# facebookresearch/actionmesh

Measured on NVIDIA H100. Metric: denoiser_steps_per_sec, higher is better.
Workload: dtype bf16

## Files before the change

actionmesh_b200/csrc/attention.cu:

```cuda
#include "common.cuh"
#include "ptx.cuh"
#include "attention.cuh"

namespace amb {

constexpr int ATT_BQ = 128;
constexpr int ATT_BK = 128;
constexpr int ATT_THREADS = 384;
constexpr int ATT_STAGES = 2;

template <int D>
struct AttnSmem {
  static constexpr int BOX_BYTES = 128 * 128;
  static constexpr int Q_BYTES = (D / 64) * BOX_BYTES;
  static constexpr int KV_BYTES = (D / 64) * BOX_BYTES;
  static constexpr int Q_OFF = 0;
  static constexpr int K_OFF = Q_BYTES;
  static constexpr int V_OFF = K_OFF + ATT_STAGES * KV_BYTES;
  static constexpr int BAR_OFF = V_OFF + ATT_STAGES * KV_BYTES;
  static constexpr int NUM_BARS = 1 + 3 * ATT_STAGES;
  static constexpr int TOTAL = BAR_OFF + NUM_BARS * 8 + 1024;
};

template <int D>
__device__ __forceinline__ void pv_k16(float* o, const uint32_t* a, uint64_t vdesc) {
  if constexpr (D == 128) wgmma_rs_n128_tb(o, a, vdesc, 1u);
  else wgmma_rs_n64_tb(o, a, vdesc, 1u);
}

template <int D>
__global__ void __launch_bounds__(ATT_THREADS, 1)
flash_attn_fwd_kernel(const __grid_constant__ CUtensorMap tmQ, const __grid_constant__ CUtensorMap tmK,
                      const __grid_constant__ CUtensorMap tmV, const AttnParams p) {
  using L = AttnSmem<D>;
  constexpr int DH = D / 64;
  extern __shared__ uint8_t smem_raw[];
  uint8_t* smem = reinterpret_cast<uint8_t*>((reinterpret_cast<uintptr_t>(smem_raw) + 1023) & ~uintptr_t(1023));
  uint64_t* q_full = reinterpret_cast<uint64_t*>(smem + L::BAR_OFF);
  uint64_t* k_full = q_full + 1;
  uint64_t* v_full = k_full + ATT_STAGES;
  uint64_t* kv_empty = v_full + ATT_STAGES;

  const int wg = __shfl_sync(0xffffffffu, threadIdx.x >> 7, 0);
  const int warp = threadIdx.x >> 5;
  const int lane = threadIdx.x & 31;
  const int q0 = blockIdx.x * ATT_BQ;
  const int head = blockIdx.y;
  const int batch = blockIdx.z;
  const int tiles_per_chunk = (p.sk_chunk + ATT_BK - 1) / ATT_BK;
  const int n_kv = p.kv_chunks * tiles_per_chunk;

  if (threadIdx.x == 0) {
    tma_prefetch_desc(&tmQ);
    tma_prefetch_desc(&tmK);
    tma_prefetch_desc(&tmV);
    mbar_init(q_full, 1);
    for (int s = 0; s < ATT_STAGES; ++s) {
      mbar_init(&k_full[s], 1);
      mbar_init(&v_full[s], 1);
      mbar_init(&kv_empty[s], 8);
    }
    fence_mbar_init();
  }
  __syncthreads();

  if (wg == 0) {
    reg_dealloc<24>();
    if (warp == 0) {
      if (elect_one()) {
        mbar_expect_tx(q_full, L::Q_BYTES);
        for (int c = 0; c < DH; ++c)
          tma_load_4d(smem + L::Q_OFF + c * L::BOX_BYTES, &tmQ, q_full, c * 64, q0, head, batch, kEvictFirst);
      }
      __syncwarp();
      int s = 0;
      uint32_t phase = 0;
      for (int j = 0; j < n_kv; ++j) {
        const int chunk = j / tiles_per_chunk;
        const int key0 = (j - chunk * tiles_per_chunk) * ATT_BK;
        mbar_wait(&kv_empty[s], phase ^ 1);
        if (elect_one()) {
          uint8_t* sk = smem + L::K_OFF + s * L::KV_BYTES;
          uint8_t* sv = smem + L::V_OFF + s * L::KV_BYTES;
          mbar_expect_tx(&k_full[s], L::KV_BYTES);
          for (int c = 0; c < DH; ++c)
            tma_load_5d(sk + c * L::BOX_BYTES, &tmK, &k_full[s], c * 64, key0, head, batch, chunk, kEvictLast);
          mbar_expect_tx(&v_full[s], L::KV_BYTES);
          for (int c = 0; c < DH; ++c)
            tma_load_5d(sv + c * L::BOX_BYTES, &tmV, &v_full[s], c * 64, key0, head, batch, chunk, kEvictLast);
        }
        __syncwarp();
        if (++s == ATT_STAGES) { s = 0; phase ^= 1; }
      }
    }
  } else {
    reg_alloc<240>();
    const int q = lane & 3;
    const int r_local = (wg - 1) * 64 + (warp & 3) * 16 + (lane >> 2);
    const uint32_t sq_addr = smem_u32(smem + L::Q_OFF) + (wg - 1) * 64 * 128;
    const uint32_t sk_addr = smem_u32(smem + L::K_OFF);
    const uint32_t sv_addr = smem_u32(smem + L::V_OFF);
    const float c = p.scale_log2;
    const int last_valid = p.sk_chunk - (tiles_per_chunk - 1) * ATT_BK;

    float o[D / 2];
#pragma unroll
    for (int i = 0; i < D / 2; ++i) o[i] = 0.f;
    float m_a = -INFINITY, m_b = -INFINITY;
    float l_a = 0.f, l_b = 0.f;

    mbar_wait(q_full, 0);
    int s = 0, jj = 0;
    uint32_t phase = 0;
    for (int j = 0; j < n_kv; ++j) {
      float sc[64];
#pragma unroll
      for (int i = 0; i < 64; ++i) sc[i] = 0.f;
      mbar_wait(&k_full[s], phase);
      wgmma_fence();
#pragma unroll
      for (int k = 0; k < D / 16; ++k) {
        const uint32_t off = (k >> 2) * L::BOX_BYTES + (k & 3) * 32;
        wgmma_ss_n128(sc, make_desc_kmajor_sw128(sq_addr + off), make_desc_kmajor_sw128(sk_addr + s * L::KV_BYTES + off), 1u);
      }
      wgmma_commit();
      wgmma_wait<0>();
#pragma unroll
      for (int i = 0; i < 64; ++i) reg_fence(sc[i]);

      if (jj == tiles_per_chunk - 1 && last_valid < ATT_BK) {
#pragma unroll
        for (int i = 0; i < 16; ++i) {
          const int key = 8 * i + 2 * q;
          if (key >= last_valid) sc[4 * i] = sc[4 * i + 2] = -INFINITY;
          if (key + 1 >= last_valid) sc[4 * i + 1] = sc[4 * i + 3] = -INFINITY;
        }
      }
      if (++jj == tiles_per_chunk) jj = 0;
      float mx_a = m_a, mx_b = m_b;
#pragma unroll
      for (int i = 0; i < 16; ++i) {
        mx_a = fmaxf(mx_a, fmaxf(sc[4 * i], sc[4 * i + 1]));
        mx_b = fmaxf(mx_b, fmaxf(sc[4 * i + 2], sc[4 * i + 3]));
      }
      mx_a = fmaxf(mx_a, __shfl_xor_sync(0xffffffffu, mx_a, 1));
      mx_b = fmaxf(mx_b, __shfl_xor_sync(0xffffffffu, mx_b, 1));
      mx_a = fmaxf(mx_a, __shfl_xor_sync(0xffffffffu, mx_a, 2));
      mx_b = fmaxf(mx_b, __shfl_xor_sync(0xffffffffu, mx_b, 2));
      const float al_a = ex2_approx((m_a - mx_a) * c), al_b = ex2_approx((m_b - mx_b) * c);
      m_a = mx_a;
      m_b = mx_b;
      const float mb_a = m_a * c, mb_b = m_b * c;
      uint32_t pk[32];
      float ts_a = 0.f, ts_b = 0.f;
#pragma unroll
      for (int i = 0; i < 16; ++i) {
        const float ea0 = ex2_approx(fmaf(sc[4 * i], c, -mb_a)), ea1 = ex2_approx(fmaf(sc[4 * i + 1], c, -mb_a));
        const float eb0 = ex2_approx(fmaf(sc[4 * i + 2], c, -mb_b)), eb1 = ex2_approx(fmaf(sc[4 * i + 3], c, -mb_b));
        ts_a += ea0 + ea1;
        ts_b += eb0 + eb1;
        pk[2 * i] = pack_bf16(ea0, ea1);
        pk[2 * i + 1] = pack_bf16(eb0, eb1);
      }
      l_a = l_a * al_a + ts_a;
      l_b = l_b * al_b + ts_b;
#pragma unroll
      for (int i = 0; i < D / 8; ++i) {
        o[4 * i] *= al_a;
        o[4 * i + 1] *= al_a;
        o[4 * i + 2] *= al_b;
        o[4 * i + 3] *= al_b;
      }

      mbar_wait(&v_full[s], phase);
      wgmma_fence();
      const uint32_t vbase = sv_addr + s * L::KV_BYTES;
#pragma unroll
      for (int kk = 0; kk < ATT_BK / 16; ++kk)
        pv_k16<D>(o, pk + 4 * kk, make_desc_mnmajor_sw128(vbase + kk * 2048, L::BOX_BYTES));
      wgmma_commit();
      wgmma_wait<0>();
#pragma unroll
      for (int i = 0; i < D / 2; ++i) reg_fence(o[i]);
      __syncwarp();
      if (lane == 0) mbar_arrive(&kv_empty[s]);
      if (++s == ATT_STAGES) { s = 0; phase ^= 1; }
    }

    l_a += __shfl_xor_sync(0xffffffffu, l_a, 1);
    l_b += __shfl_xor_sync(0xffffffffu, l_b, 1);
    l_a += __shfl_xor_sync(0xffffffffu, l_a, 2);
    l_b += __shfl_xor_sync(0xffffffffu, l_b, 2);
    const float inv_a = 1.0f / l_a, inv_b = 1.0f / l_b;
    const int qr_a = q0 + r_local, qr_b = qr_a + 8;
    __nv_bfloat16* obase = p.o + (long long)batch * p.o_stride_b + (long long)head * p.o_stride_h + 2 * q;
#pragma unroll
    for (int i = 0; i < D / 8; ++i) {
      if (qr_a < p.sq)
        *reinterpret_cast<uint32_t*>(obase + (long long)qr_a * p.o_stride_s + 8 * i) = pack_bf16(o[4 * i] * inv_a, o[4 * i + 1] * inv_a);
      if (qr_b < p.sq)
        *reinterpret_cast<uint32_t*>(obase + (long long)qr_b * p.o_stride_s + 8 * i) = pack_bf16(o[4 * i + 2] * inv_b, o[4 * i + 3] * inv_b);
    }
  }
}

template <int D>
static int launch_attn(const amb_attn_args* a, cudaStream_t stream) {
  using L = AttnSmem<D>;
  CUtensorMap tmQ, tmK, tmV;
  int r = encode_attn_maps(a, D, ATT_BQ, ATT_BK, ATT_BK, &tmQ, &tmK, &tmV);
  if (r) return r;
  const AttnParams p = make_attn_params(a);
  dim3 grid((a->sq + ATT_BQ - 1) / ATT_BQ, a->heads, a->batch);
  auto kern = flash_attn_fwd_kernel<D>;
  r = ensure_smem_optin(kern, L::TOTAL);
  if (r) return r;
  kern<<<grid, ATT_THREADS, L::TOTAL, stream>>>(tmQ, tmK, tmV, p);
  AMB_CHECK_CUDA(cudaGetLastError());
  return AMB_OK;
}

}

using namespace amb;

extern "C" int amb_flash_attn_fwd(const amb_attn_args* a, amb_stream_t stream) {
  AMB_CHECK_ARG(a && a->q && a->k && a->v && a->o, "flash_attn: null pointer");
  AMB_CHECK_ARG(a->batch > 0 && a->heads > 0 && a->sq > 0 && a->sk > 0, "flash_attn: bad shape b=%d h=%d sq=%d sk=%d",
                a->batch, a->heads, a->sq, a->sk);
  AMB_CHECK_ARG(a->head_dim == 128 || a->head_dim == 64, "flash_attn: head_dim %d unsupported (64 or 128)", a->head_dim);
  AMB_CHECK_ARG(a->q_stride_s % 8 == 0 && a->k_stride_s % 8 == 0 && a->v_stride_s % 8 == 0 && a->o_stride_s % 8 == 0 &&
                    a->q_stride_h % 8 == 0 && a->k_stride_h % 8 == 0 && a->v_stride_h % 8 == 0 && a->o_stride_h % 8 == 0 &&
                    a->q_stride_b % 8 == 0 && a->k_stride_b % 8 == 0 && a->v_stride_b % 8 == 0 && a->o_stride_b % 8 == 0,
                "flash_attn: strides must be multiples of 8 elements (16 bytes)");
  AMB_CHECK_ARG(a->kv_chunks <= 1 || (a->sk_chunk > 0 && (int64_t)a->sk_chunk * a->kv_chunks == a->sk),
                "flash_attn: kv_chunks * sk_chunk must equal sk");
  AMB_CHECK_ARG(a->batch <= 65535 && a->heads <= 65535, "flash_attn: grid limits");
  cudaStream_t s = (cudaStream_t)stream;
  if (a->head_dim == 64) return launch_attn<64>(a, s);
  return launch_attn<128>(a, s);
}
```

actionmesh_b200/csrc/ptx.cuh:

```cuda
#pragma once
#include <cstdint>
#include <cuda_runtime.h>
#include <cuda_bf16.h>

namespace amb {

__device__ __forceinline__ uint32_t smem_u32(const void* p) {
  return static_cast<uint32_t>(__cvta_generic_to_shared(p));
}
__device__ __forceinline__ uint32_t lane_id() { return threadIdx.x & 31; }

__device__ __forceinline__ bool elect_one() {
  uint32_t pred = 0;
  asm volatile(
      "{\n\t.reg .pred P;\n\t"
      "elect.sync _|P, 0xffffffff;\n\t"
      "selp.u32 %0, 1, 0, P;\n\t}\n"
      : "=r"(pred));
  return pred != 0;
}

__device__ __forceinline__ void mbar_init(uint64_t* bar, uint32_t count) {
  asm volatile("mbarrier.init.shared::cta.b64 [%0], %1;" ::"r"(smem_u32(bar)), "r"(count) : "memory");
}
__device__ __forceinline__ void fence_mbar_init() {
  asm volatile("fence.mbarrier_init.release.cluster;" ::: "memory");
}
__device__ __forceinline__ void fence_proxy_async_smem() {
  asm volatile("fence.proxy.async.shared::cta;" ::: "memory");
}
__device__ __forceinline__ void mbar_expect_tx(uint64_t* bar, uint32_t bytes) {
  asm volatile("mbarrier.arrive.expect_tx.shared::cta.b64 _, [%0], %1;" ::"r"(smem_u32(bar)), "r"(bytes)
               : "memory");
}
__device__ __forceinline__ void mbar_arrive(uint64_t* bar) {
  asm volatile("mbarrier.arrive.shared::cta.b64 _, [%0];" ::"r"(smem_u32(bar)) : "memory");
}
__device__ __forceinline__ uint32_t mbar_try_wait(uint64_t* bar, uint32_t parity) {
  uint32_t ok;
  asm volatile(
      "{\n\t.reg .pred P;\n\t"
      "mbarrier.try_wait.parity.shared::cta.b64 P, [%1], %2;\n\t"
      "selp.u32 %0, 1, 0, P;\n\t}\n"
      : "=r"(ok)
      : "r"(smem_u32(bar)), "r"(parity)
      : "memory");
  return ok;
}
__device__ __forceinline__ uint64_t globaltimer_ns() {
  uint64_t t;
  asm volatile("mov.u64 %0, %%globaltimer;" : "=l"(t));
  return t;
}
#ifndef AMB_WAIT_TIMEOUT_NS
#define AMB_WAIT_TIMEOUT_NS 4000000000ull
#endif
__device__ __forceinline__ void mbar_wait(uint64_t* bar, uint32_t parity) {
  if (mbar_try_wait(bar, parity)) return;
  uint64_t t0 = globaltimer_ns();
  uint32_t spins = 0;
  while (!mbar_try_wait(bar, parity)) {
    if ((++spins & 0xfff) == 0 && globaltimer_ns() - t0 > AMB_WAIT_TIMEOUT_NS) {
      printf("amb: mbarrier wait timeout block=(%d,%d,%d) thread=%d bar=%u parity=%u\n", blockIdx.x, blockIdx.y,
             blockIdx.z, threadIdx.x, smem_u32(bar), parity);
      __trap();
    }
  }
}

__device__ __forceinline__ void tma_prefetch_desc(const void* tmap) {
  asm volatile("prefetch.tensormap [%0];" ::"l"(reinterpret_cast<uint64_t>(tmap)) : "memory");
}
constexpr uint64_t kEvictNormal = 0x1000000000000000ull;
constexpr uint64_t kEvictFirst = 0x12F0000000000000ull;
constexpr uint64_t kEvictLast = 0x14F0000000000000ull;

__device__ __forceinline__ void tma_load_2d(void* dst, const void* tmap, uint64_t* bar, int c0, int c1,
                                            uint64_t hint) {
  asm volatile(
      "cp.async.bulk.tensor.2d.shared::cluster.global.mbarrier::complete_tx::bytes.L2::cache_hint"
      " [%0], [%1, {%3, %4}], [%2], %5;"
      :
      : "r"(smem_u32(dst)), "l"(reinterpret_cast<uint64_t>(tmap)), "r"(smem_u32(bar)), "r"(c0), "r"(c1), "l"(hint)
      : "memory");
}
__device__ __forceinline__ void tma_load_4d(void* dst, const void* tmap, uint64_t* bar, int c0, int c1, int c2,
                                            int c3, uint64_t hint) {
  asm volatile(
      "cp.async.bulk.tensor.4d.shared::cluster.global.mbarrier::complete_tx::bytes.L2::cache_hint"
      " [%0], [%1, {%3, %4, %5, %6}], [%2], %7;"
      :
      : "r"(smem_u32(dst)), "l"(reinterpret_cast<uint64_t>(tmap)), "r"(smem_u32(bar)), "r"(c0), "r"(c1), "r"(c2),
        "r"(c3), "l"(hint)
      : "memory");
}

__device__ __forceinline__ void tma_load_5d(void* dst, const void* tmap, uint64_t* bar, int c0, int c1, int c2,
                                            int c3, int c4, uint64_t hint) {
  asm volatile(
      "cp.async.bulk.tensor.5d.shared::cluster.global.mbarrier::complete_tx::bytes.L2::cache_hint"
      " [%0], [%1, {%3, %4, %5, %6, %7}], [%2], %8;"
      :
      : "r"(smem_u32(dst)), "l"(reinterpret_cast<uint64_t>(tmap)), "r"(smem_u32(bar)), "r"(c0), "r"(c1), "r"(c2),
        "r"(c3), "r"(c4), "l"(hint)
      : "memory");
}

__device__ __forceinline__ void wgmma_fence() { asm volatile("wgmma.fence.sync.aligned;" ::: "memory"); }
__device__ __forceinline__ void wgmma_commit() { asm volatile("wgmma.commit_group.sync.aligned;" ::: "memory"); }
template <int N>
__device__ __forceinline__ void wgmma_wait() {
  asm volatile("wgmma.wait_group.sync.aligned %0;" ::"n"(N) : "memory");
}
__device__ __forceinline__ void reg_fence(float& r) { asm volatile("" : "+f"(r)::"memory"); }

__device__ __forceinline__ uint64_t make_smem_desc(uint32_t saddr, uint32_t lbo_bytes, uint32_t sbo_bytes) {
  uint64_t d = 0;
  d |= static_cast<uint64_t>((saddr & 0x3FFFF) >> 4);
  d |= static_cast<uint64_t>((lbo_bytes >> 4) & 0x3FFF) << 16;
  d |= static_cast<uint64_t>((sbo_bytes >> 4) & 0x3FFF) << 32;
  d |= 1ull << 62;
  return d;
}
__device__ __forceinline__ uint64_t make_desc_kmajor_sw128(uint32_t saddr) { return make_smem_desc(saddr, 16, 1024); }
__device__ __forceinline__ uint64_t make_desc_mnmajor_sw128(uint32_t saddr, uint32_t lbo_bytes) {
  return make_smem_desc(saddr, lbo_bytes, 1024);
}

__device__ __forceinline__ void wgmma_ss_n64(float* d, uint64_t desc_a, uint64_t desc_b, uint32_t scale_d) {
  asm volatile(
      "{\n\t.reg .pred p;\n\tsetp.ne.b32 p, %34, 0;\n\t"
      "wgmma.mma_async.sync.aligned.m64n64k16.f32.bf16.bf16 {%0, %1, %2, %3, %4, %5, %6, %7, %8, %9, %10, %11, %12, %13, %14, %15, %16, %17, %18, %19, %20, %21, %22, %23, %24, %25, %26, %27, %28, %29, %30, %31}, %32, %33, p, 1, 1, 0, 0;\n\t}\n"
      : "+f"(d[0]), "+f"(d[1]), "+f"(d[2]), "+f"(d[3]), "+f"(d[4]), "+f"(d[5]), "+f"(d[6]), "+f"(d[7]), "+f"(d[8]), "+f"(d[9]), "+f"(d[10]), "+f"(d[11]), "+f"(d[12]), "+f"(d[13]), "+f"(d[14]), "+f"(d[15]), "+f"(d[16]), "+f"(d[17]), "+f"(d[18]), "+f"(d[19]), "+f"(d[20]), "+f"(d[21]), "+f"(d[22]), "+f"(d[23]), "+f"(d[24]), "+f"(d[25]), "+f"(d[26]), "+f"(d[27]), "+f"(d[28]), "+f"(d[29]), "+f"(d[30]), "+f"(d[31])
      : "l"(desc_a), "l"(desc_b), "r"(scale_d));
}
__device__ __forceinline__ void wgmma_ss_n128(float* d, uint64_t desc_a, uint64_t desc_b, uint32_t scale_d) {
  asm volatile(
      "{\n\t.reg .pred p;\n\tsetp.ne.b32 p, %66, 0;\n\t"
      "wgmma.mma_async.sync.aligned.m64n128k16.f32.bf16.bf16 {%0, %1, %2, %3, %4, %5, %6, %7, %8, %9, %10, %11, %12, %13, %14, %15, %16, %17, %18, %19, %20, %21, %22, %23, %24, %25, %26, %27, %28, %29, %30, %31, %32, %33, %34, %35, %36, %37, %38, %39, %40, %41, %42, %43, %44, %45, %46, %47, %48, %49, %50, %51, %52, %53, %54, %55, %56, %57, %58, %59, %60, %61, %62, %63}, %64, %65, p, 1, 1, 0, 0;\n\t}\n"
      : "+f"(d[0]), "+f"(d[1]), "+f"(d[2]), "+f"(d[3]), "+f"(d[4]), "+f"(d[5]), "+f"(d[6]), "+f"(d[7]), "+f"(d[8]), "+f"(d[9]), "+f"(d[10]), "+f"(d[11]), "+f"(d[12]), "+f"(d[13]), "+f"(d[14]), "+f"(d[15]), "+f"(d[16]), "+f"(d[17]), "+f"(d[18]), "+f"(d[19]), "+f"(d[20]), "+f"(d[21]), "+f"(d[22]), "+f"(d[23]), "+f"(d[24]), "+f"(d[25]), "+f"(d[26]), "+f"(d[27]), "+f"(d[28]), "+f"(d[29]), "+f"(d[30]), "+f"(d[31]), "+f"(d[32]), "+f"(d[33]), "+f"(d[34]), "+f"(d[35]), "+f"(d[36]), "+f"(d[37]), "+f"(d[38]), "+f"(d[39]), "+f"(d[40]), "+f"(d[41]), "+f"(d[42]), "+f"(d[43]), "+f"(d[44]), "+f"(d[45]), "+f"(d[46]), "+f"(d[47]), "+f"(d[48]), "+f"(d[49]), "+f"(d[50]), "+f"(d[51]), "+f"(d[52]), "+f"(d[53]), "+f"(d[54]), "+f"(d[55]), "+f"(d[56]), "+f"(d[57]), "+f"(d[58]), "+f"(d[59]), "+f"(d[60]), "+f"(d[61]), "+f"(d[62]), "+f"(d[63])
      : "l"(desc_a), "l"(desc_b), "r"(scale_d));
}
__device__ __forceinline__ void wgmma_ss_n256(float* d, uint64_t desc_a, uint64_t desc_b, uint32_t scale_d) {
  asm volatile(
      "{\n\t.reg .pred p;\n\tsetp.ne.b32 p, %130, 0;\n\t"
      "wgmma.mma_async.sync.aligned.m64n256k16.f32.bf16.bf16 {%0, %1, %2, %3, %4, %5, %6, %7, %8, %9, %10, %11, %12, %13, %14, %15, %16, %17, %18, %19, %20, %21, %22, %23, %24, %25, %26, %27, %28, %29, %30, %31, %32, %33, %34, %35, %36, %37, %38, %39, %40, %41, %42, %43, %44, %45, %46, %47, %48, %49, %50, %51, %52, %53, %54, %55, %56, %57, %58, %59, %60, %61, %62, %63, %64, %65, %66, %67, %68, %69, %70, %71, %72, %73, %74, %75, %76, %77, %78, %79, %80, %81, %82, %83, %84, %85, %86, %87, %88, %89, %90, %91, %92, %93, %94, %95, %96, %97, %98, %99, %100, %101, %102, %103, %104, %105, %106, %107, %108, %109, %110, %111, %112, %113, %114, %115, %116, %117, %118, %119, %120, %121, %122, %123, %124, %125, %126, %127}, %128, %129, p, 1, 1, 0, 0;\n\t}\n"
      : "+f"(d[0]), "+f"(d[1]), "+f"(d[2]), "+f"(d[3]), "+f"(d[4]), "+f"(d[5]), "+f"(d[6]), "+f"(d[7]), "+f"(d[8]), "+f"(d[9]), "+f"(d[10]), "+f"(d[11]), "+f"(d[12]), "+f"(d[13]), "+f"(d[14]), "+f"(d[15]), "+f"(d[16]), "+f"(d[17]), "+f"(d[18]), "+f"(d[19]), "+f"(d[20]), "+f"(d[21]), "+f"(d[22]), "+f"(d[23]), "+f"(d[24]), "+f"(d[25]), "+f"(d[26]), "+f"(d[27]), "+f"(d[28]), "+f"(d[29]), "+f"(d[30]), "+f"(d[31]), "+f"(d[32]), "+f"(d[33]), "+f"(d[34]), "+f"(d[35]), "+f"(d[36]), "+f"(d[37]), "+f"(d[38]), "+f"(d[39]), "+f"(d[40]), "+f"(d[41]), "+f"(d[42]), "+f"(d[43]), "+f"(d[44]), "+f"(d[45]), "+f"(d[46]), "+f"(d[47]), "+f"(d[48]), "+f"(d[49]), "+f"(d[50]), "+f"(d[51]), "+f"(d[52]), "+f"(d[53]), "+f"(d[54]), "+f"(d[55]), "+f"(d[56]), "+f"(d[57]), "+f"(d[58]), "+f"(d[59]), "+f"(d[60]), "+f"(d[61]), "+f"(d[62]), "+f"(d[63]), "+f"(d[64]), "+f"(d[65]), "+f"(d[66]), "+f"(d[67]), "+f"(d[68]), "+f"(d[69]), "+f"(d[70]), "+f"(d[71]), "+f"(d[72]), "+f"(d[73]), "+f"(d[74]), "+f"(d[75]), "+f"(d[76]), "+f"(d[77]), "+f"(d[78]), "+f"(d[79]), "+f"(d[80]), "+f"(d[81]), "+f"(d[82]), "+f"(d[83]), "+f"(d[84]), "+f"(d[85]), "+f"(d[86]), "+f"(d[87]), "+f"(d[88]), "+f"(d[89]), "+f"(d[90]), "+f"(d[91]), "+f"(d[92]), "+f"(d[93]), "+f"(d[94]), "+f"(d[95]), "+f"(d[96]), "+f"(d[97]), "+f"(d[98]), "+f"(d[99]), "+f"(d[100]), "+f"(d[101]), "+f"(d[102]), "+f"(d[103]), "+f"(d[104]), "+f"(d[105]), "+f"(d[106]), "+f"(d[107]), "+f"(d[108]), "+f"(d[109]), "+f"(d[110]), "+f"(d[111]), "+f"(d[112]), "+f"(d[113]), "+f"(d[114]), "+f"(d[115]), "+f"(d[116]), "+f"(d[117]), "+f"(d[118]), "+f"(d[119]), "+f"(d[120]), "+f"(d[121]), "+f"(d[122]), "+f"(d[123]), "+f"(d[124]), "+f"(d[125]), "+f"(d[126]), "+f"(d[127])
      : "l"(desc_a), "l"(desc_b), "r"(scale_d));
}
__device__ __forceinline__ void wgmma_rs_n64_tb(float* d, const uint32_t* a, uint64_t desc_b, uint32_t scale_d) {
  asm volatile(
      "{\n\t.reg .pred p;\n\tsetp.ne.b32 p, %37, 0;\n\t"
      "wgmma.mma_async.sync.aligned.m64n64k16.f32.bf16.bf16 {%0, %1, %2, %3, %4, %5, %6, %7, %8, %9, %10, %11, %12, %13, %14, %15, %16, %17, %18, %19, %20, %21, %22, %23, %24, %25, %26, %27, %28, %29, %30, %31}, {%32, %33, %34, %35}, %36, p, 1, 1, 1;\n\t}\n"
      : "+f"(d[0]), "+f"(d[1]), "+f"(d[2]), "+f"(d[3]), "+f"(d[4]), "+f"(d[5]), "+f"(d[6]), "+f"(d[7]), "+f"(d[8]), "+f"(d[9]), "+f"(d[10]), "+f"(d[11]), "+f"(d[12]), "+f"(d[13]), "+f"(d[14]), "+f"(d[15]), "+f"(d[16]), "+f"(d[17]), "+f"(d[18]), "+f"(d[19]), "+f"(d[20]), "+f"(d[21]), "+f"(d[22]), "+f"(d[23]), "+f"(d[24]), "+f"(d[25]), "+f"(d[26]), "+f"(d[27]), "+f"(d[28]), "+f"(d[29]), "+f"(d[30]), "+f"(d[31])
      : "r"(a[0]), "r"(a[1]), "r"(a[2]), "r"(a[3]), "l"(desc_b), "r"(scale_d));
}
__device__ __forceinline__ void wgmma_rs_n128_tb(float* d, const uint32_t* a, uint64_t desc_b, uint32_t scale_d) {
  asm volatile(
      "{\n\t.reg .pred p;\n\tsetp.ne.b32 p, %69, 0;\n\t"
      "wgmma.mma_async.sync.aligned.m64n128k16.f32.bf16.bf16 {%0, %1, %2, %3, %4, %5, %6, %7, %8, %9, %10, %11, %12, %13, %14, %15, %16, %17, %18, %19, %20, %21, %22, %23, %24, %25, %26, %27, %28, %29, %30, %31, %32, %33, %34, %35, %36, %37, %38, %39, %40, %41, %42, %43, %44, %45, %46, %47, %48, %49, %50, %51, %52, %53, %54, %55, %56, %57, %58, %59, %60, %61, %62, %63}, {%64, %65, %66, %67}, %68, p, 1, 1, 1;\n\t}\n"
      : "+f"(d[0]), "+f"(d[1]), "+f"(d[2]), "+f"(d[3]), "+f"(d[4]), "+f"(d[5]), "+f"(d[6]), "+f"(d[7]), "+f"(d[8]), "+f"(d[9]), "+f"(d[10]), "+f"(d[11]), "+f"(d[12]), "+f"(d[13]), "+f"(d[14]), "+f"(d[15]), "+f"(d[16]), "+f"(d[17]), "+f"(d[18]), "+f"(d[19]), "+f"(d[20]), "+f"(d[21]), "+f"(d[22]), "+f"(d[23]), "+f"(d[24]), "+f"(d[25]), "+f"(d[26]), "+f"(d[27]), "+f"(d[28]), "+f"(d[29]), "+f"(d[30]), "+f"(d[31]), "+f"(d[32]), "+f"(d[33]), "+f"(d[34]), "+f"(d[35]), "+f"(d[36]), "+f"(d[37]), "+f"(d[38]), "+f"(d[39]), "+f"(d[40]), "+f"(d[41]), "+f"(d[42]), "+f"(d[43]), "+f"(d[44]), "+f"(d[45]), "+f"(d[46]), "+f"(d[47]), "+f"(d[48]), "+f"(d[49]), "+f"(d[50]), "+f"(d[51]), "+f"(d[52]), "+f"(d[53]), "+f"(d[54]), "+f"(d[55]), "+f"(d[56]), "+f"(d[57]), "+f"(d[58]), "+f"(d[59]), "+f"(d[60]), "+f"(d[61]), "+f"(d[62]), "+f"(d[63])
      : "r"(a[0]), "r"(a[1]), "r"(a[2]), "r"(a[3]), "l"(desc_b), "r"(scale_d));
}

__device__ __forceinline__ void named_bar_sync(uint32_t id, uint32_t nthreads) {
  asm volatile("bar.sync %0, %1;" ::"r"(id), "r"(nthreads) : "memory");
}

template <int N>
__device__ __forceinline__ void reg_alloc() {
  asm volatile("setmaxnreg.inc.sync.aligned.u32 %0;" ::"n"(N));
}
template <int N>
__device__ __forceinline__ void reg_dealloc() {
  asm volatile("setmaxnreg.dec.sync.aligned.u32 %0;" ::"n"(N));
}
__device__ __forceinline__ float ex2_approx(float x) {
  float y;
  asm("ex2.approx.ftz.f32 %0, %1;" : "=f"(y) : "f"(x));
  return y;
}
__device__ __forceinline__ uint32_t pack_bf16(float lo, float hi) {
  __nv_bfloat162 v = __floats2bfloat162_rn(lo, hi);
  return *reinterpret_cast<uint32_t*>(&v);
}
__device__ __forceinline__ float2 unpack_bf16(uint32_t u) {
  __nv_bfloat162 v = *reinterpret_cast<__nv_bfloat162*>(&u);
  return __bfloat1622float2(v);
}

}
```

Measured before the change: 0.6745.

## Pipeline QK and PV wgmma across iterations with ping-pong warpgroup scheduling

```diff
diff --git a/actionmesh_b200/csrc/attention.cu b/actionmesh_b200/csrc/attention.cu
--- a/actionmesh_b200/csrc/attention.cu
+++ b/actionmesh_b200/csrc/attention.cu
@@ -18,14 +18,76 @@
   static constexpr int K_OFF = Q_BYTES;
   static constexpr int V_OFF = K_OFF + ATT_STAGES * KV_BYTES;
   static constexpr int BAR_OFF = V_OFF + ATT_STAGES * KV_BYTES;
-  static constexpr int NUM_BARS = 1 + 3 * ATT_STAGES;
+  static constexpr int NUM_BARS = 1 + 4 * ATT_STAGES;
   static constexpr int TOTAL = BAR_OFF + NUM_BARS * 8 + 1024;
 };
 
 template <int D>
-__device__ __forceinline__ void pv_k16(float* o, const uint32_t* a, uint64_t vdesc) {
-  if constexpr (D == 128) wgmma_rs_n128_tb(o, a, vdesc, 1u);
-  else wgmma_rs_n64_tb(o, a, vdesc, 1u);
+__device__ __forceinline__ void qk_issue(float* sc, uint32_t sq_addr, uint32_t sk_addr) {
+#pragma unroll
+  for (int k = 0; k < D / 16; ++k) {
+    const uint32_t off = (k >> 2) * AttnSmem<D>::BOX_BYTES + (k & 3) * 32;
+    wgmma_ss_n128(sc, make_desc_kmajor_sw128(sq_addr + off), make_desc_kmajor_sw128(sk_addr + off), k > 0 ? 1u : 0u);
+  }
+  wgmma_commit();
+}
+
+template <int D>
+__device__ __forceinline__ void pv_issue(float* o, const uint32_t* pk, uint32_t sv_addr) {
+#pragma unroll
+  for (int kk = 0; kk < ATT_BK / 16; ++kk) {
+    const uint64_t vdesc = make_desc_mnmajor_sw128(sv_addr + kk * 2048, AttnSmem<D>::BOX_BYTES);
+    if constexpr (D == 128) wgmma_rs_n128_tb(o, pk + 4 * kk, vdesc, 1u);
+    else wgmma_rs_n64_tb(o, pk + 4 * kk, vdesc, 1u);
+  }
+  wgmma_commit();
+}
+
+__device__ __forceinline__ void softmax_tile(float* sc, int valid, int q, float c, float& m_a, float& m_b, float& l_a,
+                                             float& l_b, float& al_a, float& al_b) {
+  if (valid < ATT_BK) {
+#pragma unroll
+    for (int i = 0; i < 16; ++i) {
+      const int key = 8 * i + 2 * q;
+      if (key >= valid) sc[4 * i] = sc[4 * i + 2] = -INFINITY;
+      if (key + 1 >= valid) sc[4 * i + 1] = sc[4 * i + 3] = -INFINITY;
+    }
+  }
+  float mx_a = m_a, mx_b = m_b;
+#pragma unroll
+  for (int i = 0; i < 16; ++i) {
+    mx_a = fmaxf(mx_a, fmaxf(sc[4 * i], sc[4 * i + 1]));
+    mx_b = fmaxf(mx_b, fmaxf(sc[4 * i + 2], sc[4 * i + 3]));
+  }
+  mx_a = fmaxf(mx_a, __shfl_xor_sync(0xffffffffu, mx_a, 1));
+  mx_b = fmaxf(mx_b, __shfl_xor_sync(0xffffffffu, mx_b, 1));
+  mx_a = fmaxf(mx_a, __shfl_xor_sync(0xffffffffu, mx_a, 2));
+  mx_b = fmaxf(mx_b, __shfl_xor_sync(0xffffffffu, mx_b, 2));
+  al_a = ex2_approx((m_a - mx_a) * c);
+  al_b = ex2_approx((m_b - mx_b) * c);
+  m_a = mx_a;
+  m_b = mx_b;
+  const float mb_a = m_a * c, mb_b = m_b * c;
+  float ts_a = 0.f, ts_b = 0.f;
+#pragma unroll
+  for (int i = 0; i < 16; ++i) {
+    sc[4 * i] = ex2_approx(fmaf(sc[4 * i], c, -mb_a));
+    sc[4 * i + 1] = ex2_approx(fmaf(sc[4 * i + 1], c, -mb_a));
+    sc[4 * i + 2] = ex2_approx(fmaf(sc[4 * i + 2], c, -mb_b));
+    sc[4 * i + 3] = ex2_approx(fmaf(sc[4 * i + 3], c, -mb_b));
+    ts_a += sc[4 * i] + sc[4 * i + 1];
+    ts_b += sc[4 * i + 2] + sc[4 * i + 3];
+  }
+  l_a = l_a * al_a + ts_a;
+  l_b = l_b * al_b + ts_b;
+}
+
+__device__ __forceinline__ void pack_p(uint32_t* pk, const float* sc) {
+#pragma unroll
+  for (int i = 0; i < 16; ++i) {
+    pk[2 * i] = pack_bf16(sc[4 * i], sc[4 * i + 1]);
+    pk[2 * i + 1] = pack_bf16(sc[4 * i + 2], sc[4 * i + 3]);
+  }
 }
 
 template <int D>
@@ -39,7 +101,8 @@
   uint64_t* q_full = reinterpret_cast<uint64_t*>(smem + L::BAR_OFF);
   uint64_t* k_full = q_full + 1;
   uint64_t* v_full = k_full + ATT_STAGES;
-  uint64_t* kv_empty = v_full + ATT_STAGES;
+  uint64_t* k_empty = v_full + ATT_STAGES;
+  uint64_t* v_empty = k_empty + ATT_STAGES;
 
   const int wg = __shfl_sync(0xffffffffu, threadIdx.x >> 7, 0);
   const int warp = threadIdx.x >> 5;
@@ -58,7 +121,8 @@
     for (int s = 0; s < ATT_STAGES; ++s) {
       mbar_init(&k_full[s], 1);
       mbar_init(&v_full[s], 1);
-      mbar_init(&kv_empty[s], 8);
+      mbar_init(&k_empty[s], 8);
+      mbar_init(&v_empty[s], 8);
     }
     fence_mbar_init();
   }
@@ -78,18 +142,27 @@
       for (int j = 0; j < n_kv; ++j) {
         const int chunk = j / tiles_per_chunk;
         const int key0 = (j - chunk * tiles_per_chunk) * ATT_BK;
-        mbar_wait(&kv_empty[s], phase ^ 1);
+        mbar_wait(&k_empty[s], phase ^ 1);
         if (elect_one()) {
           uint8_t* sk = smem + L::K_OFF + s * L::KV_BYTES;
-          uint8_t* sv = smem + L::V_OFF + s * L::KV_BYTES;
           mbar_expect_tx(&k_full[s], L::KV_BYTES);
           for (int c = 0; c < DH; ++c)
             tma_load_5d(sk + c * L::BOX_BYTES, &tmK, &k_full[s], c * 64, key0, head, batch, chunk, kEvictLast);
+        }
+        __syncwarp();
+        mbar_wait(&v_empty[s], phase ^ 1);
+        if (elect_one()) {
+          uint8_t* sv = smem + L::V_OFF + s * L::KV_BYTES;
           mbar_expect_tx(&v_full[s], L::KV_BYTES);
           for (int c = 0; c < DH; ++c)
             tma_load_5d(sv + c * L::BOX_BYTES, &tmV, &v_full[s], c * 64, key0, head, batch, chunk, kEvictLast);
         }
         __syncwarp();
+        if (++s == ATT_STAGES) { s = 0; phase ^= 1; }
+      }
+      for (int j = 0; j < ATT_STAGES; ++j) {
+        mbar_wait(&k_empty[s], phase ^ 1);
+        mbar_wait(&v_empty[s], phase ^ 1);
         if (++s == ATT_STAGES) { s = 0; phase ^= 1; }
       }
     }
@@ -102,68 +175,57 @@
     const uint32_t sv_addr = smem_u32(smem + L::V_OFF);
     const float c = p.scale_log2;
     const int last_valid = p.sk_chunk - (tiles_per_chunk - 1) * ATT_BK;
+    const uint32_t my_turn = wg, other_turn = 3 - wg;
 
     float o[D / 2];
 #pragma unroll
     for (int i = 0; i < D / 2; ++i) o[i] = 0.f;
     float m_a = -INFINITY, m_b = -INFINITY;
     float l_a = 0.f, l_b = 0.f;
-
-    mbar_wait(q_full, 0);
-    int s = 0, jj = 0;
+    float al_a, al_b;
+    float sc[64];
+    uint32_t pk[32];
+
+    mbar_wait_watched(q_full, 0);
+    mbar_wait_watched(&k_full[0], 0);
+    if (wg == 2) named_bar_sync(my_turn, 256);
+    wgmma_fence();
+    qk_issue<D>(sc, sq_addr, sk_addr);
+    named_bar_arrive(other_turn, 256);
+    wgmma_wait<0>();
+#pragma unroll
+    for (int i = 0; i < 64; ++i) reg_fence(sc[i]);
+    __syncwarp();
+    if (lane == 0) mbar_arrive(&k_empty[0]);
+    int jn = tiles_per_chunk == 1 ? 0 : 1;
+    softmax_tile(sc, tiles_per_chunk == 1 ? last_valid : ATT_BK, q, c, m_a, m_b, l_a, l_b, al_a, al_b);
+    pack_p(pk, sc);
+
+    int s = 0;
     uint32_t phase = 0;
-    for (int j = 0; j < n_kv; ++j) {
-      float sc[64];
-#pragma unroll
-      for (int i = 0; i < 64; ++i) sc[i] = 0.f;
-      mbar_wait(&k_full[s], phase);
+    for (int j = 0; j + 1 < n_kv; ++j) {
+      int sn = s + 1;
+      uint32_t phn = phase;
+      if (sn == ATT_STAGES) { sn = 0; phn ^= 1; }
+      mbar_wait_watched(&k_full[sn], phn);
+      mbar_wait_watched(&v_full[s], phase);
+      named_bar_sync(my_turn, 256);
       wgmma_fence();
-#pragma unroll
-      for (int k = 0; k < D / 16; ++k) {
-        const uint32_t off = (k >> 2) * L::BOX_BYTES + (k & 3) * 32;
-        wgmma_ss_n128(sc, make_desc_kmajor_sw128(sq_addr + off), make_desc_kmajor_sw128(sk_addr + s * L::KV_BYTES + off), 1u);
-      }
-      wgmma_commit();
+      qk_issue<D>(sc, sq_addr, sk_addr + sn * L::KV_BYTES);
+      pv_issue<D>(o, pk, sv_addr + s * L::KV_BYTES);
+      named_bar_arrive(other_turn, 256);
+      wgmma_wait<1>();
+#pragma unroll
+      for (int i = 0; i < 64; ++i) reg_fence(sc[i]);
+      __syncwarp();
+      if (lane == 0) mbar_arrive(&k_empty[sn]);
+      softmax_tile(sc, jn == tiles_per_chunk - 1 ? last_valid : ATT_BK, q, c, m_a, m_b, l_a, l_b, al_a, al_b);
+      if (++jn == tiles_per_chunk) jn = 0;
       wgmma_wait<0>();
 #pragma unroll
-      for (int i = 0; i < 64; ++i) reg_fence(sc[i]);
-
-      if (jj == tiles_per_chunk - 1 && last_valid < ATT_BK) {
-#pragma unroll
-        for (int i = 0; i < 16; ++i) {
-          const int key = 8 * i + 2 * q;
-          if (key >= last_valid) sc[4 * i] = sc[4 * i + 2] = -INFINITY;
-          if (key + 1 >= last_valid) sc[4 * i + 1] = sc[4 * i + 3] = -INFINITY;
-        }
-      }
-      if (++jj == tiles_per_chunk) jj = 0;
-      float mx_a = m_a, mx_b = m_b;
-#pragma unroll
-      for (int i = 0; i < 16; ++i) {
-        mx_a = fmaxf(mx_a, fmaxf(sc[4 * i], sc[4 * i + 1]));
-        mx_b = fmaxf(mx_b, fmaxf(sc[4 * i + 2], sc[4 * i + 3]));
-      }
-      mx_a = fmaxf(mx_a, __shfl_xor_sync(0xffffffffu, mx_a, 1));
-      mx_b = fmaxf(mx_b, __shfl_xor_sync(0xffffffffu, mx_b, 1));
-      mx_a = fmaxf(mx_a, __shfl_xor_sync(0xffffffffu, mx_a, 2));
-      mx_b = fmaxf(mx_b, __shfl_xor_sync(0xffffffffu, mx_b, 2));
-      const float al_a = ex2_approx((m_a - mx_a) * c), al_b = ex2_approx((m_b - mx_b) * c);
-      m_a = mx_a;
-      m_b = mx_b;
-      const float mb_a = m_a * c, mb_b = m_b * c;
-      uint32_t pk[32];
-      float ts_a = 0.f, ts_b = 0.f;
-#pragma unroll
-      for (int i = 0; i < 16; ++i) {
-        const float ea0 = ex2_approx(fmaf(sc[4 * i], c, -mb_a)), ea1 = ex2_approx(fmaf(sc[4 * i + 1], c, -mb_a));
-        const float eb0 = ex2_approx(fmaf(sc[4 * i + 2], c, -mb_b)), eb1 = ex2_approx(fmaf(sc[4 * i + 3], c, -mb_b));
-        ts_a += ea0 + ea1;
-        ts_b += eb0 + eb1;
-        pk[2 * i] = pack_bf16(ea0, ea1);
-        pk[2 * i + 1] = pack_bf16(eb0, eb1);
-      }
-      l_a = l_a * al_a + ts_a;
-      l_b = l_b * al_b + ts_b;
+      for (int i = 0; i < D / 2; ++i) reg_fence(o[i]);
+      __syncwarp();
+      if (lane == 0) mbar_arrive(&v_empty[s]);
 #pragma unroll
       for (int i = 0; i < D / 8; ++i) {
         o[4 * i] *= al_a;
@@ -171,21 +233,21 @@
         o[4 * i + 2] *= al_b;
         o[4 * i + 3] *= al_b;
       }
-
-      mbar_wait(&v_full[s], phase);
-      wgmma_fence();
-      const uint32_t vbase = sv_addr + s * L::KV_BYTES;
-#pragma unroll
-      for (int kk = 0; kk < ATT_BK / 16; ++kk)
-        pv_k16<D>(o, pk + 4 * kk, make_desc_mnmajor_sw128(vbase + kk * 2048, L::BOX_BYTES));
-      wgmma_commit();
-      wgmma_wait<0>();
-#pragma unroll
-      for (int i = 0; i < D / 2; ++i) reg_fence(o[i]);
-      __syncwarp();
-      if (lane == 0) mbar_arrive(&kv_empty[s]);
-      if (++s == ATT_STAGES) { s = 0; phase ^= 1; }
-    }
+      pack_p(pk, sc);
+      s = sn;
+      phase = phn;
+    }
+
+    mbar_wait_watched(&v_full[s], phase);
+    named_bar_sync(my_turn, 256);
+    wgmma_fence();
+    pv_issue<D>(o, pk, sv_addr + s * L::KV_BYTES);
+    if (wg == 1) named_bar_arrive(other_turn, 256);
+    wgmma_wait<0>();
+#pragma unroll
+    for (int i = 0; i < D / 2; ++i) reg_fence(o[i]);
+    __syncwarp();
+    if (lane == 0) mbar_arrive(&v_empty[s]);
 
     l_a += __shfl_xor_sync(0xffffffffu, l_a, 1);
     l_b += __shfl_xor_sync(0xffffffffu, l_b, 1);
diff --git a/actionmesh_b200/csrc/ptx.cuh b/actionmesh_b200/csrc/ptx.cuh
--- a/actionmesh_b200/csrc/ptx.cuh
+++ b/actionmesh_b200/csrc/ptx.cuh
@@ -54,6 +54,9 @@
 }
 #ifndef AMB_WAIT_TIMEOUT_NS
 #define AMB_WAIT_TIMEOUT_NS 4000000000ull
+#endif
+#ifndef AMB_WAIT_TIMEOUT_PRINT
+#define AMB_WAIT_TIMEOUT_PRINT 0
 #endif
 __device__ __forceinline__ void mbar_wait(uint64_t* bar, uint32_t parity) {
   if (mbar_try_wait(bar, parity)) return;
@@ -61,10 +64,16 @@
   uint32_t spins = 0;
   while (!mbar_try_wait(bar, parity)) {
     if ((++spins & 0xfff) == 0 && globaltimer_ns() - t0 > AMB_WAIT_TIMEOUT_NS) {
+#if AMB_WAIT_TIMEOUT_PRINT
       printf("amb: mbarrier wait timeout block=(%d,%d,%d) thread=%d bar=%u parity=%u\n", blockIdx.x, blockIdx.y,
              blockIdx.z, threadIdx.x, smem_u32(bar), parity);
+#endif
       __trap();
     }
+  }
+}
+__device__ __forceinline__ void mbar_wait_watched(uint64_t* bar, uint32_t parity) {
+  while (!mbar_try_wait(bar, parity)) {
   }
 }
 
@@ -166,6 +175,9 @@
 __device__ __forceinline__ void named_bar_sync(uint32_t id, uint32_t nthreads) {
   asm volatile("bar.sync %0, %1;" ::"r"(id), "r"(nthreads) : "memory");
 }
+__device__ __forceinline__ void named_bar_arrive(uint32_t id, uint32_t nthreads) {
+  asm volatile("bar.arrive %0, %1;" ::"r"(id), "r"(nthreads) : "memory");
+}
 
 template <int N>
 __device__ __forceinline__ void reg_alloc() {
```

New measurement: 0.7623, median of 6. +13.0%, better.
